# lunarring/latentblending

Measured on AMD Instinct MI355X. Metric: transition frames/sec, SDXL-Turbo 512x512 4-step 15-branch, higher is better.
Workload: dtype f16; 1 GPU; SDXL-Turbo 512x512, num_inference_steps=4, nmb_max_branches=15 (17 frames/transition), fp16, fixed_seeds=[420,421], anchors not recycled; frontier_width=16, hipgraphs=True, parallelism=single GPU

## Files before the change

### include/lb_hip.h

```cpp
#ifndef LB_HIP_H
#define LB_HIP_H

#include <stdint.h>

#ifdef __cplusplus
extern "C" {
#endif

typedef uint16_t lb_half;

int lb_version(void);
const char* lb_last_error_string(void);
int lb_device_info(int device, int* cu_count, long* lds_per_cu, char* arch, int arch_len);

int lb_slerp_pairs_f16(const void* const* p0, const void* const* p1, void* const* out,
                       const double* fracts, int npairs, long n, void* stream);
int lb_slerp_pairs_f32(const void* const* p0, const void* const* p1, void* const* out,
                       const double* fracts, int npairs, long n, void* stream);
int lb_slerp_pairs_f64(const void* const* p0, const void* const* p1, void* const* out,
                       const double* fracts, int npairs, long n, void* stream);
int lb_slerp_batched_f16(const void* p0, const void* p1, void* out, const double* fracts_dev,
                         long npairs, long n, void* stream);
int lb_slerp_strided_f16(const void* p0, long stride0, const void* p1, long stride1, void* out,
                         const double* fracts_dev, long npairs, long n, void* stream);
// ... 9 lines not shown
                      void* stream);
int lb_ddim_step_f16(const void* x, const void* eps, void* out, const float* params_dev, long per_sample, int batch,
                     int cfg, void* stream);

enum {
    LB_GEMM_OUT_F32 = 1,
    LB_GEMM_RES_F32 = 2,
    LB_GEMM_GEGLU = 4,
    LB_GEMM_TRANS_OUT = 8,
    LB_GEMM_SILU = 16,
    LB_GEMM_RELU = 32,
    LB_GEMM_QUICK_GELU = 128,
    LB_GEMM_GELU = 256,
    LB_GEMM_CH_STATS = 512,
    LB_GEMM_HALO_RAGGED = 1024,
    LB_GEMM_C64 = 2048,
    LB_GEMM_LN_A = 64
};

typedef struct LbGemmParams {
    const lb_half* A;
    const lb_half* W;
    void* C;
    const float* bias;
    const void* residual;
    const lb_half* rowvec;
    float* partial;
    int M, N, K;
    int lda, ldw, ldc, ldr, ld_rowvec, rows_per_batch;
    float alpha;
// ... 11 lines not shown
    float* ch_stats;
    int ch_stats_rows;
} LbGemmParams;

int lb_gemm_f16(const LbGemmParams* params, void* stream);
long lb_gemm_workspace_bytes(int M, int N);
void lb_gemm_set_tuning(int tile, int splitk);
void lb_gemm_set_pp_auto(int on);
void lb_gemm_pp_set_group(int gm);
void lb_gemm_set_depth(int depth);
int lb_gemm_plan(const LbGemmParams* p, int* tile, int* splitk, long* blocks);
int lb_conv3x3_halo_f16(const LbGemmParams* params, void* stream);
int lb_conv3x3_narrow_f16(const LbGemmParams* params, void* stream);
void lb_conv_halo_set_persistent(int on);
void lb_conv_halo_plan(const LbGemmParams* params, int* kind, int* tile_w, long* items, long* grid);
int lb_gemm_ch_stat_rows(const LbGemmParams* params);
int lb_upconv2x_halo_f16(const LbGemmParams* params, void* stream);
void lb_gemm_set_halo(int mode);
void lb_gemm_set_wide_store(int on);
void lb_gemm_set_t192_waves8(int on);
void lb_gemm_set_kgroups(int on);
void lb_gemm_set_lean_epilogue(int on);
void lb_gemm_set_variant(int variant, int stages);

void lb_groupnorm_set_l3_chunk(long bytes);
int lb_groupnorm_from_stats(const void* x, void* y, const float* gamma, const float* beta, const float* ch_stats,
                            void* workspace, int B, int HW, int C, int ldx, int ldy, int groups, float eps, int silu,
                            int x_is_f32, int stat_rows_per_sample, void* stream);
long lb_groupnorm_workspace_bytes(int B, int groups);
int lb_groupnorm_nhwc(const void* x, void* y, const float* gamma, const float* beta, void* workspace,
// ... 81 lines not shown
```

### latentblending_amd/csrc/conv3_halo.hip

```cpp
#include <type_traits>
#include "lb_common.h"
#include "lb_gemm.h"

typedef __attribute__((address_space(1))) const void* gptr_t;
typedef __attribute__((address_space(3))) void* lptr_t;

#ifndef LB_HALO_LEAN_ADDR
#define LB_HALO_LEAN_ADDR 1
#endif

template <int N> __device__ __forceinline__ void halo_wait_barrier() {
    asm volatile("s_waitcnt vmcnt(%0)\n\ts_barrier" ::"n"(N) : "memory");
}

template <int KS, int J> struct HaloSched {
    static constexpr int tap = KS == 3 ? J : (J < 3 ? 0 : 1);
};
template <int KS, int NR, int TAP> constexpr int halo_full_rounds_in_tap() {
    int n = 0;
    for (int j = 0; j < NR - 1; ++j) n += ((KS == 3 ? j : (j < 3 ? 0 : 1)) == TAP) ? 1 : 0;
    return n;
}

template <int BN, int TW, int KS = 3, bool RAG = false>
__global__ void __launch_bounds__(512) conv3x3_halo_kernel(const LbGemmParams p) {
    static_assert(!RAG || KS == 3, "ragged tiles exist for the 3x3 form only");
    constexpr int TH = 256 / TW;
    constexpr int NTAP = KS * KS;
    constexpr int HWP = TW + KS - 1;
    constexpr int HR = (TH + KS - 1) * HWP;
    constexpr int HRG = (HR + 7) / 8;
    constexpr int HRP = HRG * 8;
    constexpr int NR = (HRG + 7) / 8;
    constexpr int EXTRA = HRG - 8 * (NR - 1);
    constexpr int WI = BN * 8 / 512;
    constexpr int TM = 4, TN = BN / 32;
    static_assert(NR == (KS == 3 ? 6 : 5), "halo rounds: 6 for the 3x3 form, 5 for the 2x2 form");
    static_assert(EXTRA >= 1 && EXTRA <= 8, "the last halo round is a partial one");
    static_assert(WI == 2, "the vmcnt schedule assumes two weight loads per thread and step");
    extern __shared__ __attribute__((aligned(16))) f16 lds[];
    f16* const halo0 = lds;
// ... 1 lines not shown

    const int tid = threadIdx.x, lane = tid & 63;
    const int wave = LB_HALO_LEAN_ADDR ? __builtin_amdgcn_readfirstlane(tid >> 6) : tid >> 6;
    const int wave_m = wave >> 1, wave_n = wave & 1;
    const int g = lane >> 4, l16 = lane & 15;

    const int n_blocks = (p.N + BN - 1) / BN;
    const int tiles_x = RAG ? (p.Win + TW - 1) / TW : p.Win / TW, tiles_y = RAG ? (p.Hin + TH - 1) / TH : p.Hin / TH;
    const int n_items = (p.M / (p.Hin * p.Win)) * tiles_x * tiles_y * (KS == 2 ? 4 : 1) * n_blocks;
    const int G = gridDim.x;
    int bid = blockIdx.x;
    {
        const int q = G / 8, r = G % 8, xcd = bid % 8, idx = bid / 8;
        bid = (xcd < r ? xcd * (q + 1) : r * (q + 1) + (xcd - r) * q) + idx;
    }
    const int block_n = bid % n_blocks;
    const int par_x = KS == 2 ? (bid / n_blocks) & 1 : 0;
    const int par_y = KS == 2 ? ((bid / n_blocks) >> 1) & 1 : 0;
    const int n0 = block_n * BN;
    const int org_y = KS == 3 ? 1 : 1 - par_y, org_x = KS == 3 ? 1 : 1 - par_x;
    const lb_half* Wp = p.W + (KS == 2 ? (long)(par_y * 2 + par_x) * p.N * p.ldw : 0);
    const int nchunks = p.Cin / 64;
    const lb_half* zero = reinterpret_cast<const lb_half*>(p.zero_page);

    struct TileAt { int b, y0, x0; };
    auto tile_of = [&](int item) {
        int tile = item / n_blocks;
        if (KS == 2) tile >>= 2;
        TileAt t;
        t.x0 = (tile % tiles_x) * TW;
        tile /= tiles_x;
        t.y0 = (tile % tiles_y) * TH;
        t.b = tile / tiles_y;
        return t;
    };

    const int r8 = lane >> 3;
    const int cl = (lane & 7) ^ r8;
    long h_off[NR];
    auto set_halo_offsets = [&](const TileAt& t, bool exists) {
#pragma unroll
        for (int j = 0; j < NR; ++j) {
            const int gidx = j * 8 + wave;
            const int row = gidx * 8 + r8;
            const int hy = row / HWP, hx = row - hy * HWP;
            const int y = t.y0 + hy - org_y, x = t.x0 + hx - org_x;
            const bool ok = exists && (j < NR - 1 || wave < EXTRA) && row < HR && y >= 0 && y < p.Hin && x >= 0 && x < p.Win;
            h_off[j] = ok ? ((long)(t.b * p.Hin + y) * p.Win + x) * p.ldx + cl * 8 : -1;
        }
    };
    long w_off[WI];
    unsigned w_off32[WI];
#pragma unroll
    for (int i = 0; i < WI; ++i) {
        const int n = n0 + (tid >> 3) + i * 64;
        w_off[i] = n < p.N ? (long)n * p.ldw + cl * 8 : -1;
        w_off32[i] = (unsigned)(((long)(n < p.N ? n : p.N - 1) * p.ldw + cl * 8) * 2);
    }

#ifdef LB_STUDY_BUILD
    const int study = p.reserved_;
#else
    constexpr int study = 0;
#endif
    auto issue_halo = [&](int j, int src_chunk, int buf) {
        const lb_half* src = h_off[j] >= 0 && !(study & 2) ? p.A + h_off[j] + (long)src_chunk * 64 : zero;
        const int gidx = j * 8 + wave;
        f16* dst = halo0 + buf * (HRP * 64) + gidx * 8 * 64;
        __builtin_amdgcn_global_load_lds((gptr_t)src, (lptr_t)dst, 16, 0, 0);
    };
    auto issue_weight = [&](int i, int chunk, bool exists, int tap, int slot) {
        f16* dst = wring + slot * (BN * 64) + (wave * 8 + i * 64) * 64;
        if constexpr (LB_HALO_LEAN_ADDR) {
            if (!(study & 4)) {
                const char* base = reinterpret_cast<const char*>(Wp) + ((long)tap * p.Cin + (long)chunk * 64) * 2;
                __builtin_amdgcn_global_load_lds((gptr_t)(base + (size_t)w_off32[i]), (lptr_t)dst, 16, 0, 0);
                return;
            }
        }
        const bool live = w_off[i] >= 0 && exists && !(study & 4);
        const lb_half* src = live ? Wp + w_off[i] + (long)tap * p.Cin + (long)chunk * 64 : zero;
        __builtin_amdgcn_global_load_lds((gptr_t)src, (lptr_t)dst, 16, 0, 0);
    };

    int hbase[TM];
    int mloc[TM];
#pragma unroll
    for (int i = 0; i < TM; ++i) {
        const int m = wave_m * 64 + i * 16 + l16;
        const int py = m / TW, px = m - py * TW;
        hbase[i] = py * HWP + px;
        mloc[i] = py * p.Win + px;
    }
    f32x4 acc[TM][TN];
#pragma unroll
    for (int i = 0; i < TM; ++i)
// ... 20 lines not shown
        }
#pragma unroll
        for (int j = 0; j < TN; ++j) {
            const int r = j * 16 + l16;
            wf[j] = *reinterpret_cast<const f16x8*>(wb + (wave_n * (BN / 2) + r) * 64 + ((chunk ^ (r & 7)) << 3));
        }
    };
    auto mma_rows = [&](const f16x8 (&af)[TM], const f16x8 (&wf)[TN], int i_lo, int i_hi) {
#pragma unroll
        for (int i = i_lo; i < i_hi; ++i)
#pragma unroll
            for (int j = 0; j < TN; ++j)
                acc[i][j] = __builtin_amdgcn_mfma_f32_16x16x32_f16(wf[j], af[i], acc[i][j], 0, 0, 0);
    };

    int item = bid;
    TileAt cur = tile_of(item);
    set_halo_offsets(cur, true);
#pragma unroll
    for (int j = 0; j < NR; ++j)
        if (j < NR - 1 || wave < EXTRA) issue_halo(j, 0, 0);
#pragma unroll
    for (int t = 0; t < 3; ++t)
#pragma unroll
        for (int i = 0; i < WI; ++i) issue_weight(i, 0, true, t, t);

    auto step = [&](auto tap_c, int c, int cc, bool more) {
        constexpr int TAP = decltype(tap_c)::value;
        constexpr int P1 = (TAP + NTAP - 1) % NTAP, P2 = (TAP + NTAP - 2) % NTAP;
        constexpr int CNT = (2 + halo_full_rounds_in_tap<KS, NR, P1>()) + (2 + halo_full_rounds_in_tap<KS, NR, P2>());
        halo_wait_barrier<CNT>();
        const int slot = KS == 3 ? ((cc + TAP) & 3) : TAP;
        const f16* hb = halo0 + (cc & 1) * (HRP * 64);
        const f16* wb = wring + slot * (BN * 64);
        constexpr int KY = TAP / KS, KX = TAP % KS;
        int shift = KY * HWP + KX;
        asm volatile("" : "+v"(shift));
        const bool last = c + 1 == nchunks;
        const int hc = last ? 0 : c + 1, hbuf = (cc + 1) & 1;
        constexpr int TAP3 = (TAP + 3) % NTAP;
        const bool wrap = (TAP + 3 >= NTAP) && last;
        const int c3 = wrap ? 0 : c + (TAP + 3) / NTAP;
        const bool w_exists = !wrap || more;
        const int slot3 = (slot + 3) & 3;
        f16x8 a0[TM], w0[TN], a1[TM], w1[TN];
        read_frags(hb, wb, shift, 0, a0, w0);
        if constexpr (HaloSched<KS, 0>::tap == TAP) issue_halo(0, hc, hbuf);
        if constexpr (NR > 2 && HaloSched<KS, 1>::tap == TAP) issue_halo(1, hc, hbuf);
        if constexpr (NR > 3 && HaloSched<KS, 2>::tap == TAP) issue_halo(2, hc, hbuf);
        if constexpr (NR > 4 && HaloSched<KS, 3>::tap == TAP) { if (NR - 1 > 3 || wave < EXTRA) issue_halo(3, hc, hbuf); }
        if constexpr (NR > 4 && HaloSched<KS, 4>::tap == TAP) { if (NR - 1 > 4 || wave < EXTRA) issue_halo(4, hc, hbuf); }
        if constexpr (NR > 5 && HaloSched<KS, 5>::tap == TAP) { if (wave < EXTRA) issue_halo(5, hc, hbuf); }
        __builtin_amdgcn_sched_barrier(0);
        mma_rows(a0, w0, 0, TM / 2);
        read_frags(hb, wb, shift, 1, a1, w1);
        __builtin_amdgcn_sched_barrier(0);
        issue_weight(0, c3, w_exists, TAP3, slot3);
        __builtin_amdgcn_sched_barrier(0);
        mma_rows(a0, w0, TM / 2, TM);
        __builtin_amdgcn_sched_barrier(0);
        issue_weight(1, c3, w_exists, TAP3, slot3);
        __builtin_amdgcn_sched_barrier(0);
        mma_rows(a1, w1, 0, TM);
    };

    LbGemmParams q = p;
    if constexpr (KS == 2) {
        q.scatter = 1;
        q.sc_py = par_y;
        q.sc_px = par_x;
    }

    int cc = 0;
    for (;;) {
        const int next_item = item + G;
        const bool more = next_item < n_items;
        const TileAt nxt = tile_of(more ? next_item : item);
        for (int c = 0; c < nchunks; ++c, ++cc) {
            if (c + 1 == nchunks) set_halo_offsets(nxt, more);
            step(std::integral_constant<int, 0>{}, c, cc, more);
            step(std::integral_constant<int, 1>{}, c, cc, more);
            step(std::integral_constant<int, 2>{}, c, cc, more);
            step(std::integral_constant<int, 3>{}, c, cc, more);
            if constexpr (KS == 3) {
                step(std::integral_constant<int, 4>{}, c, cc, more);
                step(std::integral_constant<int, 5>{}, c, cc, more);
                step(std::integral_constant<int, 6>{}, c, cc, more);
                step(std::integral_constant<int, 7>{}, c, cc, more);
                step(std::integral_constant<int, 8>{}, c, cc, more);
            }
        }
        const int mbase = (cur.b * p.Hin + cur.y0) * p.Win + cur.x0;
        int col0 = n0 + wave_n * (BN / 2) + 4 * g;
        asm volatile("" : "+v"(col0));
        bool overhang = false;
        if constexpr (RAG) overhang = cur.y0 + TH > p.Hin || cur.x0 + TW > p.Win;
        if (RAG && overhang && !(study & 1)) {
            int tid_o = tid;
            asm volatile("" : "+v"(tid_o));
            auto row_of = [&](int i) {
                const int ml = (tid_o >> 7) * 64 + i * 16 + (tid_o & 15), ly = ml / TW, lx = ml - ly * TW;
                return cur.y0 + ly < p.Hin && cur.x0 + lx < p.Win ? mbase + mloc[i] : p.M;
            };
            if (p.flags & LB_GEMM_CH_STATS) {
                const long stat_rows = (long)(n_items / n_blocks) * 4;
                float2* chst = reinterpret_cast<float2*>(p.ch_stats) + ((long)(item / n_blocks) * 4 + wave_m);
                lb_gemm_tile_epilogue_rows_ln<TM, TN, false, false, true, true>(q, acc, row_of, col0, 0, (const LbLnRows<TM>*)nullptr, chst, stat_rows);
            } else {
                lb_gemm_tile_epilogue_rows<TM, TN, false>(q, acc, row_of, col0, 0);
            }
        } else if (!(study & 1)) {
            int tid_o = tid;
            asm volatile("" : "+v"(tid_o));
            auto out_rel = [&](int i) {
                if constexpr (KS == 3) return mloc[i];
                const int ml = (tid_o >> 7) * 64 + i * 16 + (tid_o & 15), ly = ml / TW, lx = ml - ly * TW;
                return 4 * ly * p.Win + 2 * lx;
            };
            const long out_lo = KS == 3 ? (long)mbase
                                        : ((long)(cur.b * 2 * p.Hin + 2 * cur.y0 + par_y)) * (2 * p.Win) + 2 * cur.x0 + par_x;
            const int row_hi = mbase + (TH - 1) * p.Win + TW;
            const int colw = col0 - 4 * ((tid_o & 63) >> 4);
            if (p.flags & LB_GEMM_CH_STATS) {
                const long stat_rows = (long)(n_items / n_blocks) * 4;
                float2* chst = reinterpret_cast<float2*>(p.ch_stats) + ((long)(item / n_blocks) * 4 + wave_m);
                if (!lb_gemm_tile_epilogue_lean<TM, TN, true, true>(q, acc, [&](int i) { return mbase + mloc[i]; }, mbase, row_hi, out_rel,
                                                                    out_lo, cur.b, colw, chst, stat_rows))
                    lb_gemm_tile_epilogue_rows_ln<TM, TN, false, false, true>(q, acc, [&](int i) { return mbase + mloc[i]; }, col0, 0,
                                                                              (const LbLnRows<TM>*)nullptr, chst, stat_rows);
            } else {
                if (!lb_gemm_tile_epilogue_lean<TM, TN, false, true>(q, acc, [&](int i) { return mbase + mloc[i]; }, mbase, row_hi, out_rel,
                                                                     out_lo, cur.b, colw))
                    lb_gemm_tile_epilogue_rows<TM, TN, false>(q, acc, [&](int i) { return mbase + mloc[i]; }, col0, 0);
            }
        }
        else if (acc[0][0][0] == 12345.678f) *(float*)p.C = acc[1][1][1] + acc[2][2][2] + acc[3][3][3];
        if (!more) break;
#pragma unroll
        for (int i = 0; i < TM; ++i)
#pragma unroll
            for (int j = 0; j < TN; ++j) acc[i][j] = (f32x4){0.f, 0.f, 0.f, 0.f};
        item = next_item;
        cur = nxt;
    }
    asm volatile("s_waitcnt vmcnt(0)" ::: "memory");
}

static int g_halo_persistent = 1;
extern "C" void lb_conv_halo_set_persistent(int on) { g_halo_persistent = on; }
#ifdef LB_STUDY_BUILD
static int g_halo_study = 0;
extern "C" void lb_conv_halo_set_study(int bits) { g_halo_study = bits; }
#endif
static int halo_num_cus() {
    static int n = 0;
    if (!n) {
        int dev = 0;
        hipDeviceProp_t prop;
// ... 14 lines not shown
        grid = (long)(halo_num_cus() / period) * period;
}

int lb_upconv_halo_eligible(const LbGemmParams& p);
int lb_conv3x3_halo_eligible(const LbGemmParams& p);
long lb_conv_halo_stat_rows_total(const LbGemmParams& p) {
    int tw = 0, ks = 0;
    if ((tw = lb_upconv_halo_eligible(p)) != 0) ks = 2;
    else if ((tw = lb_conv3x3_halo_eligible(p)) != 0) ks = 3;
    if (!ks) return 0;
    long items, grid;
    halo_grid(p, tw, ks, items, grid);
    return items / ((p.N + 127) / 128) * 4;
}

template <int BN, int TW, int KS = 3, bool RAG = false>
static int launch_halo(const LbGemmParams& p, hipStream_t stream) {
    constexpr int TH = 256 / TW;
    constexpr int HRP = (((TH + KS - 1) * (TW + KS - 1) + 7) / 8) * 8;
    constexpr int SMEM = (2 * HRP * 64 + 4 * BN * 64) * (int)sizeof(f16);
    static unsigned long long seen = 0;
    LB_ONCE_PER_DEVICE(seen)
        (void)hipFuncSetAttribute(reinterpret_cast<const void*>(conv3x3_halo_kernel<BN, TW, KS, RAG>),
                                  hipFuncAttributeMaxDynamicSharedMemorySize, SMEM);
    static_assert(BN == 128, "halo_grid assumes 128-channel blocks");
    long nblk, grid;
    halo_grid(p, TW, KS, nblk, grid);
    LbGemmParams pk = p;
#ifdef LB_STUDY_BUILD
    pk.reserved_ = g_halo_study;
#endif
    hipLaunchKernelGGL((conv3x3_halo_kernel<BN, TW, KS, RAG>), dim3((unsigned)grid), dim3(512), SMEM, stream, pk);
    return lb_check_launch(KS == 2 ? "lb_upconv2x_halo_f16" : "lb_conv3x3_halo_f16");
}

int lb_upconv_halo_eligible(const LbGemmParams& p) {
    if (!p.conv || p.scatter != 2 || p.KH != 2 || p.KW != 2 || p.stride != 1 || p.ups) return 0;
    if (p.Hout != p.Hin || p.Wout != p.Win || p.Cin % 64 != 0 || p.K != 4 * p.Cin) return 0;
    if (p.zero_page == nullptr || (p.flags & (LB_GEMM_GEGLU | LB_GEMM_TRANS_OUT)) || p.N % 4 != 0 || p.residual != nullptr) return 0;
    if (p.M % (p.Hin * p.Win) != 0) return 0;
    if ((long)p.N * p.ldw * 2 >= (1l << 32)) return 0;
    if (p.Win % 32 == 0 && p.Hin % 8 == 0) return 32;
    if (p.Win % 16 == 0 && p.Hin % 16 == 0) return 16;
    return 0;
}

static int halo_tiles_check(const LbGemmParams& p, int tw, int ks) {
// ... 30 lines not shown

int lb_conv3x3_halo_eligible(const LbGemmParams& p) {
    if (!p.conv || p.KH != 3 || p.KW != 3 || p.stride != 1 || p.pad != 1 || p.ups || p.scatter) return 0;
    if (p.Hout != p.Hin || p.Wout != p.Win || p.Cin % 64 != 0 || p.K != 9 * p.Cin) return 0;
    if (p.zero_page == nullptr || (p.flags & LB_GEMM_GEGLU) || p.N % 4 != 0) return 0;
    if (p.M % (p.Hin * p.Win) != 0) return 0;
    if ((long)p.N * p.ldw * 2 >= (1l << 32)) return 0;
    if (p.Win % 32 == 0 && p.Hin % 8 == 0) return 32;
    if (p.Win % 16 == 0 && p.Hin % 16 == 0) return 16;
    if (!(p.flags & LB_GEMM_HALO_RAGGED)) return 0;
    const long t32 = (long)((p.Win + 31) / 32) * ((p.Hin + 7) / 8), t16 = (long)((p.Win + 15) / 16) * ((p.Hin + 15) / 16);
    return t16 < t32 ? 16 : 32;
}
static bool halo3_ragged(const LbGemmParams& p, int tw) { return p.Win % tw != 0 || p.Hin % (256 / tw) != 0; }

long lb_conv3x3_halo_blocks(const LbGemmParams& p) {
    long tiles = (long)p.M / 256;
    if (const int tw = (p.flags & LB_GEMM_HALO_RAGGED) ? lb_conv3x3_halo_eligible(p) : 0)
        tiles = (long)(p.M / (p.Hin * p.Win)) * ((p.Hin + 256 / tw - 1) / (256 / tw)) * ((p.Win + tw - 1) / tw);
    return tiles * ((p.N + 127) / 128);
}

int lb_conv3x3_halo_check(const LbGemmParams& p) {
    LB_REQUIRE(!(p.flags & LB_GEMM_CH_STATS) || (p.ch_stats != nullptr && !(p.flags & LB_GEMM_TRANS_OUT)),
               "halo conv: LB_GEMM_CH_STATS needs ch_stats and a row-major output");
    LB_REQUIRE(!(p.flags & LB_GEMM_CH_STATS) || p.ch_stats_rows == lb_conv_halo_stat_rows_total(p),
               "halo conv: ch_stats_rows must be B * lb_gemm_ch_stat_rows() (the row blocks this launch writes per channel)");
    return halo_tiles_check(p, lb_conv3x3_halo_eligible(p), 3);
}

int lb_conv3x3_halo_launch(LbGemmParams p, hipStream_t stream) {
    if (p.alpha == 0.f) p.alpha = 1.f;
    p.splitk = 1;
    const int tw = lb_conv3x3_halo_eligible(p);
    if (halo3_ragged(p, tw)) return tw == 32 ? launch_halo<128, 32, 3, true>(p, stream) : launch_halo<128, 16, 3, true>(p, stream);
    return tw == 32 ? launch_halo<128, 32>(p, stream) : launch_halo<128, 16>(p, stream);
}

extern "C" int lb_conv3x3_halo_f16(const LbGemmParams* pp, void* stream) {
    LbGemmParams p = *pp;
    p.flags &= ~LB_GEMM_C64;
    p.reserved2_ = (g_lb_wide_store & 1) | (g_lb_lean_epilogue ? 2 : 0);
    LB_REQUIRE(p.M > 0 && p.N > 0 && p.K > 0, "lb_conv3x3_halo_f16: empty problem");
    LB_REQUIRE(lb_conv3x3_halo_eligible(p) != 0,
               "lb_conv3x3_halo_f16: needs a 3x3 / stride 1 / pad 1 conv, Cin % 64 == 0, W % 16 == 0 (or LB_GEMM_HALO_RAGGED), zero page");
    LB_REQUIRE(p.ldw % 8 == 0 && p.ldx % 8 == 0 && (p.ldc % 4 == 0 || (p.flags & LB_GEMM_TRANS_OUT)),
               "lb_conv3x3_halo_f16: ldw / ldx multiples of 8, ldc multiple of 4");
    if (const int rc = lb_conv3x3_halo_check(p)) return rc;
    LB_DISPATCH("lb_conv3x3_halo_f16", lb_conv3x3_halo_launch(p, s));
}
// ... 15 lines not shown
```

### latentblending_amd/csrc/gemm.hip

```cpp
#include "lb_common.h"
#include "lb_gemm.h"

#define BK 64

template <int N> struct Int { static constexpr int value = N; };

template <int BM, int BN, bool CONV, bool GEGLU, int D>
__global__ void __launch_bounds__(256) gemm_f16_kernel(const LbGemmParams p) {
    constexpr int AI = BM * 8 / 256;
    constexpr int WI = BN * 8 / 256;
    constexpr int TM = BM / 32;
    constexpr int TN = BN / 32;
    __shared__ __attribute__((aligned(16))) f16 lds[2 * (BM + BN) * BK];
    f16* const As = lds;
    f16* const Ws = lds + 2 * BM * BK;

    const int tid = threadIdx.x;
    const int lane = tid & 63, wave = tid >> 6;
    const int wave_m = wave >> 1, wave_n = wave & 1;
    const int g = lane >> 4, l16 = lane & 15;

    const int n_blocks = GEGLU ? (p.N / 2 + BN / 2 - 1) / (BN / 2) : (p.N + BN - 1) / BN;
    int bid = blockIdx.x;
    {
// ... 471 lines not shown
        LB_DISPATCH("conv3x3_c64", lb_conv3_c64_launch(p, s));
    }
    if (p.scatter == 2) {
        LB_REQUIRE(lb_upconv_halo_eligible(p) != 0, "lb_gemm_f16: scatter = 2 needs Cin % 64 == 0, W % 16 == 0, stacked [4][N][K] weights");
        if (const int rc = lb_upconv_halo_check(p)) return rc;
        LB_DISPATCH("lb_upconv2x_halo_f16", lb_upconv_halo_launch(p, s));
    }
    if (g_halo != 0 && !g_force_tile && lb_conv3x3_narrow_eligible(p)) {
        if (const int rc = lb_conv3x3_narrow_check(p)) return rc;
        LB_DISPATCH("lb_conv3x3_narrow_f16", lb_conv3x3_narrow_launch(p, s));
    }
    if (use_halo(p)) {
        if (const int rc = lb_conv3x3_halo_check(p)) return rc;
        LB_DISPATCH("lb_conv3x3_halo_f16", lb_conv3x3_halo_launch(p, s));
    }
    LB_REQUIRE(!(p.flags & LB_GEMM_CH_STATS), "lb_gemm_f16: LB_GEMM_CH_STATS is implemented by the halo-tile conv kernels only "
                                              "(check lb_gemm_plan == 6 / lb_conv_halo_plan before asking for it)");
    int tile = 0, splitk = 1;
    long nblk = 0;
    gemm_plan(p, tile, splitk, nblk);
    p.splitk = splitk;
    const int depth = g_depth, variant = g_variant;
    int stages = g_stages;
    if (variant == 1) {
        lb_gemm_glds_init();
        if (stages == 0)
            stages = (tile == 3 || tile == 4 || tile == 7 || tile == 10 || tile == 11) ? 3 : 2;
    }
    const dim3 grid((unsigned)nblk, 1, (unsigned)splitk);
    LB_DISPATCH("lb_gemm_f16", gemm_launch_impl(p, tile, depth, variant, stages, grid, s));
// ... 2 lines not shown
```

### latentblending_amd/hip/lib.py

```python
from __future__ import annotations

import ctypes as C
import os

import torch

_HERE = os.path.dirname(os.path.abspath(__file__))
LIB_PATH = os.environ.get("LB_HIP_LIBRARY") or os.path.join(_HERE, "liblbhip.so")

c_void_pp = C.POINTER(C.c_void_p)


class LbGemmParams(C.Structure):
    _fields_ = [
        ("A", C.c_void_p), ("W", C.c_void_p), ("C", C.c_void_p), ("bias", C.c_void_p),
        ("residual", C.c_void_p), ("rowvec", C.c_void_p), ("partial", C.c_void_p),
        ("M", C.c_int), ("N", C.c_int), ("K", C.c_int),
        ("lda", C.c_int), ("ldw", C.c_int), ("ldc", C.c_int), ("ldr", C.c_int),
        ("ld_rowvec", C.c_int), ("rows_per_batch", C.c_int),
        ("alpha", C.c_float), ("flags", C.c_int),
        ("conv", C.c_int), ("Hin", C.c_int), ("Win", C.c_int), ("Cin", C.c_int),
        ("Hout", C.c_int), ("Wout", C.c_int), ("KH", C.c_int), ("KW", C.c_int),
        ("stride", C.c_int), ("pad", C.c_int), ("ups", C.c_int), ("ldx", C.c_int),
        ("splitk", C.c_int), ("zero_page", C.c_void_p),
# ... 2 lines not shown
    ]


class LbAttnParams(C.Structure):
    _fields_ = [
        ("Q", C.c_void_p), ("K", C.c_void_p), ("V", C.c_void_p), ("O", C.c_void_p),
        ("B", C.c_int), ("H", C.c_int), ("Sq", C.c_int), ("Skv", C.c_int), ("Skv_valid", C.c_int),
        ("ldq", C.c_int), ("ldk", C.c_int), ("ldv", C.c_int), ("ldo", C.c_int),
        ("scale", C.c_float), ("causal", C.c_int), ("zero_page", C.c_void_p), ("reserved_", C.c_int),
    ]


GEMM_OUT_F32, GEMM_RES_F32, GEMM_GEGLU, GEMM_TRANS_OUT, GEMM_SILU, GEMM_RELU, GEMM_LN_A = 1, 2, 4, 8, 16, 32, 64
GEMM_QUICK_GELU, GEMM_GELU, GEMM_CH_STATS = 128, 256, 512
GEMM_HALO_RAGGED = 1024
GEMM_C64 = 2048

_vp, _i, _l, _f, _d = C.c_void_p, C.c_int, C.c_long, C.c_float, C.c_double

SIGNATURES = {
    "lb_version": (_i, []),
    "lb_last_error_string": (C.c_char_p, []),
    "lb_device_info": (_i, [_i, C.POINTER(_i), C.POINTER(_l), C.c_char_p, _i]),
    "lb_slerp_pairs_f16": (_i, [c_void_pp, c_void_pp, c_void_pp, C.POINTER(_d), _i, _l, _vp]),
    "lb_slerp_pairs_f32": (_i, [c_void_pp, c_void_pp, c_void_pp, C.POINTER(_d), _i, _l, _vp]),
    "lb_slerp_pairs_f64": (_i, [c_void_pp, c_void_pp, c_void_pp, C.POINTER(_d), _i, _l, _vp]),
    "lb_slerp_batched_f16": (_i, [_vp, _vp, _vp, _vp, _l, _l, _vp]),
    "lb_slerp_strided_f16": (_i, [_vp, _l, _vp, _l, _vp, _vp, _l, _l, _vp]),
    "lb_lerp_f16": (_i, [_vp, _vp, _vp, _l, _d, _vp]),
    "lb_lerp_f32": (_i, [_vp, _vp, _vp, _l, _d, _vp]),
# ... 59 lines not shown
    "lb_program_num_ops": (_i, [_vp]),
    "lb_program_op_name": (C.c_char_p, [_vp, _i]),
    "lb_program_run": (_i, [_vp, _vp]),
    "lb_program_run_range": (_i, [_vp, _i, _i, _vp]),
    "lb_program_instantiate": (_i, [_vp]),
    "lb_program_launch": (_i, [_vp, _vp]),
    "lb_program_time_ops": (_i, [_vp, _vp, C.POINTER(C.c_float)]),
}

STUDY_SIGNATURES = {
    "lb_slerp_set_study": (None, [_i]),
    "lb_gemm_set_policy": (None, [_i]),
    "lb_conv_halo_set_study": (None, [_i]),
}

_NO_CHECK = {"lb_version", "lb_last_error_string", "lb_gemm_workspace_bytes", "lb_jpeg_coefficient_count", "lb_jpeg_workspace_bytes",
             "lb_groupnorm_workspace_bytes", "lb_groupnorm_set_l3_chunk", "lb_conv_halo_set_persistent", "lb_conv_halo_plan", "lb_gemm_ch_stat_rows", "lb_conv_halo_set_study", "lb_gemm_set_tuning", "lb_gemm_set_depth", "lb_gemm_set_variant", "lb_gemm_set_wide_store", "lb_gemm_set_lean_epilogue", "lb_gemm_set_t192_waves8", "lb_gemm_set_kgroups", "lb_gemm_pp_set_group", "lb_gemm_set_pp_auto", "lb_gemm_set_policy", "lb_gemm_set_halo", "lb_attn_set_tuning", "lb_layernorm_set_form", "lb_groupnorm_set_fused", "lb_groupnorm_plan", "lb_slerp_set_study", "lb_program_create",
             "lb_program_destroy", "lb_program_recording", "lb_program_num_ops", "lb_program_op_name"}


def _load():
    if not os.path.isfile(LIB_PATH):
        raise ImportError(
            f"latentblending_amd: {LIB_PATH} is missing. Build it with "
            "`python -c 'import __graft_entry__ as g; g.build()'` (hipcc, gfx950). "
            "There is no CPU fallback for the kernel path.")
    return C.CDLL(LIB_PATH, mode=C.RTLD_GLOBAL)


_lib = _load()


# ... 6 lines not shown
        rc = fn(*args)
        if rc != 0:
            msg = _lib.lb_last_error_string()
            raise RuntimeError(f"{name} failed ({rc}): {msg.decode() if msg else '?'}")
        return rc
    checked.__name__ = name
    return checked


api = _Api()
for _name, (_res, _args) in SIGNATURES.items():
    _fn = getattr(_lib, _name)
    _fn.restype = _res
    _fn.argtypes = _args
    setattr(api, _name, _fn if _name in _NO_CHECK else _wrap(_name, _fn))
for _name, (_res, _args) in STUDY_SIGNATURES.items():
    _fn = getattr(_lib, _name, None)
    if _fn is not None:
        _fn.restype = _res
        _fn.argtypes = _args
        setattr(api, _name, _fn)

if os.environ.get("LB_GEMM_WIDE_STORE"):
    api.lb_gemm_set_wide_store(int(os.environ["LB_GEMM_WIDE_STORE"]))
if os.environ.get("LB_GEMM_LEAN_EPILOGUE"):
    api.lb_gemm_set_lean_epilogue(int(os.environ["LB_GEMM_LEAN_EPILOGUE"]))
if os.environ.get("LB_GEMM_PP_AUTO"):
    api.lb_gemm_set_pp_auto(int(os.environ["LB_GEMM_PP_AUTO"]))
```

### latentblending_amd/native/runtime.py

```python
from __future__ import annotations

import contextlib
import ctypes as C
from typing import Dict, List, Optional, Tuple

import torch

from ..hip import lib
from ..hip.lib import api, LbGemmParams, LbAttnParams
from .geometry import use_ragged_halo

F16, F32 = torch.float16, torch.float32


class Arena:
    def __init__(self, device):
        self.device = device
        self.free: Dict[int, List[torch.Tensor]] = {}
        self.all: List[torch.Tensor] = []
        self.bytes_allocated = 0

    @staticmethod
    def _cls(nbytes: int) -> int:
        return max(512, (nbytes + 511) // 512 * 512)
# ... 89 lines not shown


class Emitter:

    def __init__(self, arena: Arena):
        self.arena = arena
        self.device = arena.device
        self.ws_gemm: Optional[torch.Tensor] = None
        self.ws_gn: Optional[torch.Tensor] = None
        self.gemm_log: List[dict] = []
        self.attn_log: List[dict] = []
        self.norm_log: List[dict] = []
        self._retired: List[torch.Tensor] = []
        self.zero_page = torch.zeros(64, dtype=torch.uint8, device=self.device)
        self.ragged_halo = False

    def _ragged_flag(self, p: LbGemmParams) -> int:
        if not self.ragged_halo or not p.conv or p.KH != 3 or p.KW != 3 or p.stride != 1 or p.scatter or p.ups or p.N <= 16:
            return 0
        kind, tw = C.c_int(), C.c_int()
        flags = p.flags
        p.flags = flags & ~lib.GEMM_HALO_RAGGED
        api.lb_conv_halo_plan(C.byref(p), C.byref(kind), None, None, None)
        plain = kind.value
        p.flags = flags | lib.GEMM_HALO_RAGGED
        api.lb_conv_halo_plan(C.byref(p), C.byref(kind), C.byref(tw), None, None)
        p.flags = flags
        return lib.GEMM_HALO_RAGGED if use_ragged_halo(True, plain, kind.value, p.Hin, p.Win, tw.value) else 0

    def _gemm_ws(self, M: int, N: int) -> Optional[torch.Tensor]:
        if ((M + 63) // 64) * ((N + 63) // 64) > 640:
            return None
        need = api.lb_gemm_workspace_bytes(M, N) // 4
        if self.ws_gemm is None or self.ws_gemm.numel() < need:
            if self.ws_gemm is not None:
                self._retired.append(self.ws_gemm)
            self.ws_gemm = torch.empty(max(need, 1 << 22), dtype=F32, device=self.device)
        return self.ws_gemm

    def _gn_ws(self, B: int, groups: int) -> torch.Tensor:
        need = api.lb_groupnorm_workspace_bytes(B, groups) // 8
        if self.ws_gn is None or self.ws_gn.numel() < need:
            if self.ws_gn is not None:
                self._retired.append(self.ws_gn)
            self.ws_gn = torch.empty(need, dtype=torch.float64, device=self.device)
        return self.ws_gn

    def gemm(self, A: torch.Tensor, W: torch.Tensor, out: torch.Tensor, *, M: int, bias=None,
             residual=None, rowvec=None, rows_per_batch: int = 0, flags: int = 0, alpha: float = 1.0,
             lda: Optional[int] = None, ldc: Optional[int] = None, ldr: Optional[int] = None,
             ld_rowvec: Optional[int] = None, conv: Optional[dict] = None, splitk: bool = True,
             ln: Optional[Tuple[torch.Tensor, float]] = None, ch_stats: Optional[torch.Tensor] = None):
        p = LbGemmParams()
# ... 17 lines not shown
        if rowvec is not None:
            p.ld_rowvec, p.rows_per_batch = ld_rowvec if ld_rowvec is not None else N, rows_per_batch
        p.alpha, p.flags = alpha, flags
        p.zero_page = self.zero_page.data_ptr()
        if ln is not None:
            p.flags |= lib.GEMM_LN_A
            p.ln_colsum, p.ln_eps = ln[0].data_ptr(), float(ln[1])
        if ch_stats is not None:
            assert conv is not None and ch_stats.dtype == F32
            p.flags |= lib.GEMM_CH_STATS
            p.ch_stats, p.ch_stats_rows = ch_stats.data_ptr(), ch_stats.shape[1]
        if splitk and not (flags & lib.GEMM_GEGLU) and ln is None:
            p.partial = _p(self._gemm_ws(M, N))
        if self.ragged_halo:
            p.flags |= self._ragged_flag(p)
        api.lb_gemm_f16(C.byref(p), _stream())
        mult = 4.0 if p.scatter == 2 else 1.0
        self.gemm_log.append({"M": M, "N": N, "K": K, "flops": mult * 2.0 * M * N * K, "conv": conv is not None,
                              "bytes": mult * 2.0 * (N * K + M * n_out) + (2.0 * M * K if conv is None else 0.0)})
        return out

    def plan(self, M: int, N: int, K: int, flags: int = 0) -> Tuple[int, int]:
        p = LbGemmParams()
        p.M, p.N, p.K, p.flags = M, N, K, flags
        p.zero_page = self.zero_page.data_ptr()
        if not (flags & lib.GEMM_GEGLU):
            p.partial = _p(self._gemm_ws(M, N))
        t, sk, nb = C.c_int(), C.c_int(), C.c_long()
        api.lb_gemm_plan(C.byref(p), C.byref(t), C.byref(sk), C.byref(nb))
        return t.value, sk.value
# ... 62 lines not shown
```

Before: 124.1 frames/s.

## Add stream-K style split of the input-channel loop for halo 3x3 convs

Adds a K-split variant of the persistent halo 3x3 conv kernel. Work is divided into (tile, 64-channel chunk) units spread evenly over a CU-sized grid. Blocks that hold a partial tile write fp32 accumulators to slabs and bump an atomic counter, and the last block to arrive reduces the slabs and runs the epilogue. The goal is to remove tail-wave load imbalance when the number of tiles does not divide evenly across CUs. The cost is extra slab traffic, atomics and a fixup reduction, and a host-side plan decides per conv whether splitting is worth it.

New measurement: 126.1 frames/s, median of 6. +1.6%, better.

```diff
diff --git a/include/lb_hip.h b/include/lb_hip.h
--- a/include/lb_hip.h
+++ b/include/lb_hip.h
@@ -47,6 +47,7 @@
     LB_GEMM_GELU = 256,
     LB_GEMM_CH_STATS = 512,
     LB_GEMM_HALO_RAGGED = 1024,
+    LB_GEMM_HALO_KSPLIT = 4096,
     LB_GEMM_C64 = 2048,
     LB_GEMM_LN_A = 64
 };
@@ -88,6 +89,7 @@
 int lb_conv3x3_narrow_f16(const LbGemmParams* params, void* stream);
 void lb_conv_halo_set_persistent(int on);
 void lb_conv_halo_plan(const LbGemmParams* params, int* kind, int* tile_w, long* items, long* grid);
+#include "lb_hip_ksplit.h"
 int lb_gemm_ch_stat_rows(const LbGemmParams* params);
 int lb_upconv2x_halo_f16(const LbGemmParams* params, void* stream);
 void lb_gemm_set_halo(int mode);
diff --git a/include/lb_hip_ksplit.h b/include/lb_hip_ksplit.h
--- /dev/null
+++ b/include/lb_hip_ksplit.h
@@ -0,0 +1,12 @@
+#ifndef LB_HIP_KSPLIT_H
+#define LB_HIP_KSPLIT_H
+#ifdef __cplusplus
+extern "C" {
+#endif
+void lb_conv_halo_ksplit_plan(const LbGemmParams* params, long* units, long* grid, int* split);
+long lb_conv_halo_ksplit_workspace_bytes(const LbGemmParams* params);
+void lb_conv_halo_set_ksplit(int mode, int grid);
+#ifdef __cplusplus
+}
+#endif
+#endif
diff --git a/latentblending_amd/csrc/conv3_halo.hip b/latentblending_amd/csrc/conv3_halo.hip
--- a/latentblending_amd/csrc/conv3_halo.hip
+++ b/latentblending_amd/csrc/conv3_halo.hip
@@ -22,9 +22,10 @@
     return n;
 }
 
-template <int BN, int TW, int KS = 3, bool RAG = false>
+template <int BN, int TW, int KS = 3, bool RAG = false, bool KSP = false>
 __global__ void __launch_bounds__(512) conv3x3_halo_kernel(const LbGemmParams p) {
     static_assert(!RAG || KS == 3, "ragged tiles exist for the 3x3 form only");
+    static_assert(!KSP || (KS == 3 && !RAG), "the K-split form exists for the whole-tile 3x3 form only");
     constexpr int TH = 256 / TW;
     constexpr int NTAP = KS * KS;
     constexpr int HWP = TW + KS - 1;
@@ -56,10 +57,16 @@
         const int q = G / 8, r = G % 8, xcd = bid % 8, idx = bid / 8;
         bid = (xcd < r ? xcd * (q + 1) : r * (q + 1) + (xcd - r) * q) + idx;
     }
-    const int block_n = bid % n_blocks;
+    const int n_tiles = KSP ? n_items / n_blocks : 0;
+    const long n_units = KSP ? (long)n_items * (p.Cin / 64) : 0;
+    const long u_lo = KSP ? (long)bid * n_units / G : 0, u_hi = KSP ? (long)(bid + 1) * n_units / G : 0;
+    if constexpr (KSP)
+        if (u_lo >= u_hi) return;
+    const int first_item = KSP ? (int)(u_lo / (p.Cin / 64)) : bid;
+    const int block_n = KSP ? first_item / n_tiles : bid % n_blocks;
     const int par_x = KS == 2 ? (bid / n_blocks) & 1 : 0;
     const int par_y = KS == 2 ? ((bid / n_blocks) >> 1) & 1 : 0;
-    const int n0 = block_n * BN;
+    int n0 = block_n * BN;
     const int org_y = KS == 3 ? 1 : 1 - par_y, org_x = KS == 3 ? 1 : 1 - par_x;
     const lb_half* Wp = p.W + (KS == 2 ? (long)(par_y * 2 + par_x) * p.N * p.ldw : 0);
     const int nchunks = p.Cin / 64;
@@ -67,7 +74,7 @@
 
     struct TileAt { int b, y0, x0; };
     auto tile_of = [&](int item) {
-        int tile = item / n_blocks;
+        int tile = KSP ? item % n_tiles : item / n_blocks;
         if (KS == 2) tile >>= 2;
         TileAt t;
         t.x0 = (tile % tiles_x) * TW;
@@ -91,14 +98,18 @@
             h_off[j] = ok ? ((long)(t.b * p.Hin + y) * p.Win + x) * p.ldx + cl * 8 : -1;
         }
     };
-    long w_off[WI];
-    unsigned w_off32[WI];
-#pragma unroll
-    for (int i = 0; i < WI; ++i) {
-        const int n = n0 + (tid >> 3) + i * 64;
-        w_off[i] = n < p.N ? (long)n * p.ldw + cl * 8 : -1;
-        w_off32[i] = (unsigned)(((long)(n < p.N ? n : p.N - 1) * p.ldw + cl * 8) * 2);
-    }
+    long w_off[WI], w_offn[WI];
+    unsigned w_off32[WI], w_off32n[WI];
+    auto set_w_offsets = [&](int col_base, long (&o64)[WI], unsigned (&o32)[WI]) {
+#pragma unroll
+        for (int i = 0; i < WI; ++i) {
+            const int n = col_base + (tid >> 3) + i * 64;
+            o64[i] = n < p.N ? (long)n * p.ldw + cl * 8 : -1;
+            o32[i] = (unsigned)(((long)(n < p.N ? n : p.N - 1) * p.ldw + cl * 8) * 2);
+        }
+    };
+    set_w_offsets(n0, w_off, w_off32);
+    if constexpr (KSP) set_w_offsets(n0, w_offn, w_off32n);
 
 #ifdef LB_STUDY_BUILD
     const int study = p.reserved_;
@@ -111,17 +122,19 @@
         f16* dst = halo0 + buf * (HRP * 64) + gidx * 8 * 64;
         __builtin_amdgcn_global_load_lds((gptr_t)src, (lptr_t)dst, 16, 0, 0);
     };
-    auto issue_weight = [&](int i, int chunk, bool exists, int tap, int slot) {
+    auto issue_weight = [&](int i, int chunk, bool exists, int tap, int slot, bool nxt_slab = false) {
         f16* dst = wring + slot * (BN * 64) + (wave * 8 + i * 64) * 64;
         if constexpr (LB_HALO_LEAN_ADDR) {
             if (!(study & 4)) {
                 const char* base = reinterpret_cast<const char*>(Wp) + ((long)tap * p.Cin + (long)chunk * 64) * 2;
-                __builtin_amdgcn_global_load_lds((gptr_t)(base + (size_t)w_off32[i]), (lptr_t)dst, 16, 0, 0);
+                const unsigned o32 = KSP && nxt_slab ? w_off32n[i] : w_off32[i];
+                __builtin_amdgcn_global_load_lds((gptr_t)(base + (size_t)o32), (lptr_t)dst, 16, 0, 0);
                 return;
             }
         }
-        const bool live = w_off[i] >= 0 && exists && !(study & 4);
-        const lb_half* src = live ? Wp + w_off[i] + (long)tap * p.Cin + (long)chunk * 64 : zero;
+        const long o64 = KSP && nxt_slab ? w_offn[i] : w_off[i];
+        const bool live = o64 >= 0 && exists && !(study & 4);
+        const lb_half* src = live ? Wp + o64 + (long)tap * p.Cin + (long)chunk * 64 : zero;
         __builtin_amdgcn_global_load_lds((gptr_t)src, (lptr_t)dst, 16, 0, 0);
     };
 
@@ -172,16 +185,21 @@
                 acc[i][j] = __builtin_amdgcn_mfma_f32_16x16x32_f16(wf[j], af[i], acc[i][j], 0, 0, 0);
     };
 
-    int item = bid;
+    int item = first_item;
+    int c_lo = 0, c_end = nchunks;
+    if constexpr (KSP) {
+        c_lo = (int)(u_lo - (long)item * nchunks);
+        c_end = (int)(u_hi - (long)item * nchunks < nchunks ? u_hi - (long)item * nchunks : nchunks);
+    }
     TileAt cur = tile_of(item);
     set_halo_offsets(cur, true);
 #pragma unroll
     for (int j = 0; j < NR; ++j)
-        if (j < NR - 1 || wave < EXTRA) issue_halo(j, 0, 0);
+        if (j < NR - 1 || wave < EXTRA) issue_halo(j, c_lo, 0);
 #pragma unroll
     for (int t = 0; t < 3; ++t)
 #pragma unroll
-        for (int i = 0; i < WI; ++i) issue_weight(i, 0, true, t, t);
+        for (int i = 0; i < WI; ++i) issue_weight(i, c_lo, true, t, t);
 
     auto step = [&](auto tap_c, int c, int cc, bool more) {
         constexpr int TAP = decltype(tap_c)::value;
@@ -194,7 +212,7 @@
         constexpr int KY = TAP / KS, KX = TAP % KS;
         int shift = KY * HWP + KX;
         asm volatile("" : "+v"(shift));
-        const bool last = c + 1 == nchunks;
+        const bool last = c + 1 == c_end;
         const int hc = last ? 0 : c + 1, hbuf = (cc + 1) & 1;
         constexpr int TAP3 = (TAP + 3) % NTAP;
         const bool wrap = (TAP + 3 >= NTAP) && last;
@@ -213,11 +231,11 @@
         mma_rows(a0, w0, 0, TM / 2);
         read_frags(hb, wb, shift, 1, a1, w1);
         __builtin_amdgcn_sched_barrier(0);
-        issue_weight(0, c3, w_exists, TAP3, slot3);
+        issue_weight(0, c3, w_exists, TAP3, slot3, wrap);
         __builtin_amdgcn_sched_barrier(0);
         mma_rows(a0, w0, TM / 2, TM);
         __builtin_amdgcn_sched_barrier(0);
-        issue_weight(1, c3, w_exists, TAP3, slot3);
+        issue_weight(1, c3, w_exists, TAP3, slot3, wrap);
         __builtin_amdgcn_sched_barrier(0);
         mma_rows(a1, w1, 0, TM);
     };
@@ -231,11 +249,15 @@
 
     int cc = 0;
     for (;;) {
-        const int next_item = item + G;
-        const bool more = next_item < n_items;
+        const int next_item = KSP ? item + 1 : item + G;
+        const bool more = KSP ? (long)next_item * nchunks < u_hi : next_item < n_items;
         const TileAt nxt = tile_of(more ? next_item : item);
-        for (int c = 0; c < nchunks; ++c, ++cc) {
-            if (c + 1 == nchunks) set_halo_offsets(nxt, more);
+        const int n0_next = KSP && more ? (next_item / n_tiles) * BN : n0;
+        for (int c = c_lo; c < c_end; ++c, ++cc) {
+            if (c + 1 == c_end) {
+                set_halo_offsets(nxt, more);
+                if constexpr (KSP) set_w_offsets(n0_next, w_offn, w_off32n);
+            }
             step(std::integral_constant<int, 0>{}, c, cc, more);
             step(std::integral_constant<int, 1>{}, c, cc, more);
             step(std::integral_constant<int, 2>{}, c, cc, more);
@@ -246,6 +268,68 @@
                 step(std::integral_constant<int, 6>{}, c, cc, more);
                 step(std::integral_constant<int, 7>{}, c, cc, more);
                 step(std::integral_constant<int, 8>{}, c, cc, more);
+            }
+        }
+        if constexpr (KSP) {
+            if (c_lo != 0 || c_end != nchunks) {
+                const long t0 = (long)item * nchunks;
+                const int b_first = (int)(((t0 + 1) * G - 1) / n_units), b_last = (int)(((t0 + nchunks) * G - 1) / n_units);
+                constexpr long SLAB = 256l * BN;
+                int* const counters = reinterpret_cast<int*>(p.partial);
+                float* const slabs = p.partial + (((long)n_items * 4 + 255) / 256) * 64;
+                int tid_s = tid;
+                asm volatile("" : "+v"(tid_s));
+                typedef unsigned u32x4 __attribute__((ext_vector_type(4)));
+                const __amdgpu_buffer_rsrc_t srs = __builtin_amdgcn_make_buffer_rsrc(slabs, 0, (int)(unsigned)(2l * G * SLAB * 4), 0x00020000);
+                const int voff = tid_s * 16;
+                const int mine = (2 * bid + (item == first_item ? 0 : 1)) * (int)(SLAB * 4);
+#pragma unroll
+                for (int i = 0; i < TM; ++i)
+#pragma unroll
+                    for (int j = 0; j < TN; ++j)
+                        __builtin_amdgcn_raw_buffer_store_b128(__builtin_bit_cast(u32x4, acc[i][j]), srs, voff, mine + (i * TN + j) * 8192, 16);
+                volatile int* const flag = reinterpret_cast<volatile int*>(lds + 2 * HRP * 64 + 4 * BN * 64);
+                asm volatile("s_waitcnt vmcnt(0)" ::: "memory");
+                __syncthreads();
+                if (tid == 0) {
+                    const int ticket = __hip_atomic_fetch_add(counters + item, 1, __ATOMIC_RELAXED, __HIP_MEMORY_SCOPE_AGENT);
+                    const bool last_one = ticket == b_last - b_first;
+                    if (last_one) __hip_atomic_store(counters + item, 0, __ATOMIC_RELAXED, __HIP_MEMORY_SCOPE_AGENT);
+                    *flag = last_one ? 1 : 0;
+                }
+                __syncthreads();
+                const bool reduce = __builtin_amdgcn_readfirstlane(*flag) != 0;
+                if (!reduce) {
+                    if (!more) break;
+#pragma unroll
+                    for (int i = 0; i < TM; ++i)
+#pragma unroll
+                        for (int j = 0; j < TN; ++j) acc[i][j] = (f32x4){0.f, 0.f, 0.f, 0.f};
+                    item = next_item;
+                    cur = nxt;
+                    n0 = n0_next;
+                    set_w_offsets(n0, w_off, w_off32);
+                    c_lo = 0;
+                    c_end = (int)(u_hi - (long)item * nchunks < nchunks ? u_hi - (long)item * nchunks : nchunks);
+                    continue;
+                }
+#pragma unroll
+                for (int i = 0; i < TM; ++i)
+#pragma unroll
+                    for (int j = 0; j < TN; ++j) acc[i][j] = (f32x4){0.f, 0.f, 0.f, 0.f};
+                for (int b = b_first; b <= b_last; ++b) {
+                    const bool first_tile_of_b = (long)b * n_units / G / nchunks == item;
+                    const int src = (2 * b + (first_tile_of_b ? 0 : 1)) * (int)(SLAB * 4);
+#pragma unroll
+                    for (int i = 0; i < TM; ++i) {
+                        f32x4 part[TN];
+#pragma unroll
+                        for (int j = 0; j < TN; ++j)
+                            part[j] = __builtin_bit_cast(f32x4, __builtin_amdgcn_raw_buffer_load_b128(srs, voff, src + (i * TN + j) * 8192, 16));
+#pragma unroll
+                        for (int j = 0; j < TN; ++j) acc[i][j] += part[j];
+                    }
+                }
             }
         }
         const int mbase = (cur.b * p.Hin + cur.y0) * p.Win + cur.x0;
@@ -262,7 +346,7 @@
             };
             if (p.flags & LB_GEMM_CH_STATS) {
                 const long stat_rows = (long)(n_items / n_blocks) * 4;
-                float2* chst = reinterpret_cast<float2*>(p.ch_stats) + ((long)(item / n_blocks) * 4 + wave_m);
+                float2* chst = reinterpret_cast<float2*>(p.ch_stats) + ((long)(KSP ? item % n_tiles : item / n_blocks) * 4 + wave_m);
                 lb_gemm_tile_epilogue_rows_ln<TM, TN, false, false, true, true>(q, acc, row_of, col0, 0, (const LbLnRows<TM>*)nullptr, chst, stat_rows);
             } else {
                 lb_gemm_tile_epilogue_rows<TM, TN, false>(q, acc, row_of, col0, 0);
@@ -281,7 +365,7 @@
             const int colw = col0 - 4 * ((tid_o & 63) >> 4);
             if (p.flags & LB_GEMM_CH_STATS) {
                 const long stat_rows = (long)(n_items / n_blocks) * 4;
-                float2* chst = reinterpret_cast<float2*>(p.ch_stats) + ((long)(item / n_blocks) * 4 + wave_m);
+                float2* chst = reinterpret_cast<float2*>(p.ch_stats) + ((long)(KSP ? item % n_tiles : item / n_blocks) * 4 + wave_m);
                 if (!lb_gemm_tile_epilogue_lean<TM, TN, true, true>(q, acc, [&](int i) { return mbase + mloc[i]; }, mbase, row_hi, out_rel,
                                                                     out_lo, cur.b, colw, chst, stat_rows))
                     lb_gemm_tile_epilogue_rows_ln<TM, TN, false, false, true>(q, acc, [&](int i) { return mbase + mloc[i]; }, col0, 0,
@@ -300,6 +384,12 @@
             for (int j = 0; j < TN; ++j) acc[i][j] = (f32x4){0.f, 0.f, 0.f, 0.f};
         item = next_item;
         cur = nxt;
+        if constexpr (KSP) {
+            n0 = n0_next;
+            set_w_offsets(n0, w_off, w_off32);
+            c_lo = 0;
+            c_end = (int)(u_hi - (long)item * nchunks < nchunks ? u_hi - (long)item * nchunks : nchunks);
+        }
     }
     asm volatile("s_waitcnt vmcnt(0)" ::: "memory");
 }
@@ -344,23 +434,24 @@
     return items / ((p.N + 127) / 128) * 4;
 }
 
-template <int BN, int TW, int KS = 3, bool RAG = false>
-static int launch_halo(const LbGemmParams& p, hipStream_t stream) {
+template <int BN, int TW, int KS = 3, bool RAG = false, bool KSP = false>
+static int launch_halo(const LbGemmParams& p, hipStream_t stream, long ksp_grid = 0) {
     constexpr int TH = 256 / TW;
     constexpr int HRP = (((TH + KS - 1) * (TW + KS - 1) + 7) / 8) * 8;
-    constexpr int SMEM = (2 * HRP * 64 + 4 * BN * 64) * (int)sizeof(f16);
+    constexpr int SMEM = (2 * HRP * 64 + 4 * BN * 64) * (int)sizeof(f16) + (KSP ? 16 : 0);
     static unsigned long long seen = 0;
     LB_ONCE_PER_DEVICE(seen)
-        (void)hipFuncSetAttribute(reinterpret_cast<const void*>(conv3x3_halo_kernel<BN, TW, KS, RAG>),
+        (void)hipFuncSetAttribute(reinterpret_cast<const void*>(conv3x3_halo_kernel<BN, TW, KS, RAG, KSP>),
                                   hipFuncAttributeMaxDynamicSharedMemorySize, SMEM);
     static_assert(BN == 128, "halo_grid assumes 128-channel blocks");
     long nblk, grid;
     halo_grid(p, TW, KS, nblk, grid);
+    if (KSP) grid = ksp_grid;
     LbGemmParams pk = p;
 #ifdef LB_STUDY_BUILD
     pk.reserved_ = g_halo_study;
 #endif
-    hipLaunchKernelGGL((conv3x3_halo_kernel<BN, TW, KS, RAG>), dim3((unsigned)grid), dim3(512), SMEM, stream, pk);
+    hipLaunchKernelGGL((conv3x3_halo_kernel<BN, TW, KS, RAG, KSP>), dim3((unsigned)grid), dim3(512), SMEM, stream, pk);
     return lb_check_launch(KS == 2 ? "lb_upconv2x_halo_f16" : "lb_conv3x3_halo_f16");
 }
 
@@ -421,6 +512,55 @@
 }
 static bool halo3_ragged(const LbGemmParams& p, int tw) { return p.Win % tw != 0 || p.Hin % (256 / tw) != 0; }
 
+static int g_halo_ksplit_mode = 1, g_halo_ksplit_grid = 0;
+extern "C" void lb_conv_halo_set_ksplit(int mode, int grid) {
+    g_halo_ksplit_mode = mode < 0 ? 1 : mode;
+    g_halo_ksplit_grid = grid > 0 ? grid : 0;
+}
+static constexpr long HALO_KSPLIT_FIXUP_STEPS = 20;
+static constexpr long HALO_KSPLIT_MARGIN_PCT = 5;
+static void halo_ksplit_plan(const LbGemmParams& p, long& units, long& grid, int& split) {
+    units = grid = 0;
+    split = 0;
+    if (!(p.flags & LB_GEMM_HALO_KSPLIT) || (p.flags & LB_GEMM_C64) || g_halo_ksplit_mode == 0) return;
+    const int tw = lb_conv3x3_halo_eligible(p);
+    if (!tw || halo3_ragged(p, tw) || p.Cin < 128) return;
+    long items, ugrid;
+    halo_grid(p, tw, 3, items, ugrid);
+    const long nchunks = p.Cin / 64;
+    if (items * nchunks >= (1l << 31)) return;
+    units = items * nchunks;
+    grid = g_halo_ksplit_grid > 0 ? g_halo_ksplit_grid : halo_num_cus();
+    if (grid > units) grid = units;
+    if (2 * grid * 256l * 128 * 4 >= (1l << 31)) {
+        units = grid = 0;
+        return;
+    }
+    if (g_halo_ksplit_mode >= 2) {
+        split = 1;
+        return;
+    }
+    const long unsplit_steps = (items + ugrid - 1) / ugrid * 9 * nchunks;
+    const long split_steps = (units + grid - 1) / grid * 9 + HALO_KSPLIT_FIXUP_STEPS;
+    split = split_steps * (100 + HALO_KSPLIT_MARGIN_PCT) <= unsplit_steps * 100 ? 1 : 0;
+}
+static long halo_ksplit_counter_bytes(long items) { return (items * 4 + 255) / 256 * 256; }
+extern "C" void lb_conv_halo_ksplit_plan(const LbGemmParams* pp, long* units, long* grid, int* split) {
+    long u = 0, g = 0;
+    int s = 0;
+    if (pp != nullptr && pp->M > 0 && pp->Hin > 0 && pp->Win > 0) halo_ksplit_plan(*pp, u, g, s);
+    if (units) *units = u;
+    if (grid) *grid = g;
+    if (split) *split = s;
+}
+extern "C" long lb_conv_halo_ksplit_workspace_bytes(const LbGemmParams* pp) {
+    long u = 0, g = 0;
+    int s = 0;
+    if (pp != nullptr && pp->M > 0 && pp->Hin > 0 && pp->Win > 0) halo_ksplit_plan(*pp, u, g, s);
+    if (!s) return 0;
+    return halo_ksplit_counter_bytes(u / (pp->Cin / 64)) + 2 * g * 256l * 128 * (long)sizeof(float);
+}
+
 long lb_conv3x3_halo_blocks(const LbGemmParams& p) {
     long tiles = (long)p.M / 256;
     if (const int tw = (p.flags & LB_GEMM_HALO_RAGGED) ? lb_conv3x3_halo_eligible(p) : 0)
@@ -433,6 +573,13 @@
                "halo conv: LB_GEMM_CH_STATS needs ch_stats and a row-major output");
     LB_REQUIRE(!(p.flags & LB_GEMM_CH_STATS) || p.ch_stats_rows == lb_conv_halo_stat_rows_total(p),
                "halo conv: ch_stats_rows must be B * lb_gemm_ch_stat_rows() (the row blocks this launch writes per channel)");
+    {
+        long units, grid;
+        int split;
+        halo_ksplit_plan(p, units, grid, split);
+        LB_REQUIRE(!split || p.partial != nullptr,
+                   "halo conv: LB_GEMM_HALO_KSPLIT needs partial = a zeroed workspace of lb_conv_halo_ksplit_workspace_bytes()");
+    }
     return halo_tiles_check(p, lb_conv3x3_halo_eligible(p), 3);
 }
 
@@ -441,6 +588,11 @@
     p.splitk = 1;
     const int tw = lb_conv3x3_halo_eligible(p);
     if (halo3_ragged(p, tw)) return tw == 32 ? launch_halo<128, 32, 3, true>(p, stream) : launch_halo<128, 16, 3, true>(p, stream);
+    long units, grid;
+    int split;
+    halo_ksplit_plan(p, units, grid, split);
+    if (split && p.partial != nullptr)
+        return tw == 32 ? launch_halo<128, 32, 3, false, true>(p, stream, grid) : launch_halo<128, 16, 3, false, true>(p, stream, grid);
     return tw == 32 ? launch_halo<128, 32>(p, stream) : launch_halo<128, 16>(p, stream);
 }
 
diff --git a/latentblending_amd/csrc/gemm.hip b/latentblending_amd/csrc/gemm.hip
--- a/latentblending_amd/csrc/gemm.hip
+++ b/latentblending_amd/csrc/gemm.hip
@@ -509,6 +509,10 @@
         if (const int rc = lb_conv3x3_halo_check(p)) return rc;
         LB_DISPATCH("lb_conv3x3_halo_f16", lb_conv3x3_halo_launch(p, s));
     }
+    if (p.flags & LB_GEMM_HALO_KSPLIT) {
+        p.flags &= ~LB_GEMM_HALO_KSPLIT;
+        p.partial = nullptr;
+    }
     LB_REQUIRE(!(p.flags & LB_GEMM_CH_STATS), "lb_gemm_f16: LB_GEMM_CH_STATS is implemented by the halo-tile conv kernels only "
                                               "(check lb_gemm_plan == 6 / lb_conv_halo_plan before asking for it)");
     int tile = 0, splitk = 1;
diff --git a/latentblending_amd/hip/lib.py b/latentblending_amd/hip/lib.py
--- a/latentblending_amd/hip/lib.py
+++ b/latentblending_amd/hip/lib.py
@@ -40,6 +40,7 @@
 GEMM_OUT_F32, GEMM_RES_F32, GEMM_GEGLU, GEMM_TRANS_OUT, GEMM_SILU, GEMM_RELU, GEMM_LN_A = 1, 2, 4, 8, 16, 32, 64
 GEMM_QUICK_GELU, GEMM_GELU, GEMM_CH_STATS = 128, 256, 512
 GEMM_HALO_RAGGED = 1024
+GEMM_HALO_KSPLIT = 4096
 GEMM_C64 = 2048
 
 _vp, _i, _l, _f, _d = C.c_void_p, C.c_int, C.c_long, C.c_float, C.c_double
@@ -129,8 +130,14 @@
     "lb_conv_halo_set_study": (None, [_i]),
 }
 
+HOST_SIGNATURES = {
+    "lb_conv_halo_ksplit_plan": (None, [C.POINTER(LbGemmParams), C.POINTER(C.c_long), C.POINTER(C.c_long), C.POINTER(C.c_int)]),
+    "lb_conv_halo_ksplit_workspace_bytes": (_l, [C.POINTER(LbGemmParams)]),
+    "lb_conv_halo_set_ksplit": (None, [_i, _i]),
+}
+
 _NO_CHECK = {"lb_version", "lb_last_error_string", "lb_gemm_workspace_bytes", "lb_jpeg_coefficient_count", "lb_jpeg_workspace_bytes",
-             "lb_groupnorm_workspace_bytes", "lb_groupnorm_set_l3_chunk", "lb_conv_halo_set_persistent", "lb_conv_halo_plan", "lb_gemm_ch_stat_rows", "lb_conv_halo_set_study", "lb_gemm_set_tuning", "lb_gemm_set_depth", "lb_gemm_set_variant", "lb_gemm_set_wide_store", "lb_gemm_set_lean_epilogue", "lb_gemm_set_t192_waves8", "lb_gemm_set_kgroups", "lb_gemm_pp_set_group", "lb_gemm_set_pp_auto", "lb_gemm_set_policy", "lb_gemm_set_halo", "lb_attn_set_tuning", "lb_layernorm_set_form", "lb_groupnorm_set_fused", "lb_groupnorm_plan", "lb_slerp_set_study", "lb_program_create",
+             "lb_groupnorm_workspace_bytes", "lb_groupnorm_set_l3_chunk", "lb_conv_halo_set_persistent", "lb_conv_halo_plan","lb_gemm_ch_stat_rows", "lb_conv_halo_set_study", "lb_gemm_set_tuning", "lb_gemm_set_depth", "lb_gemm_set_variant", "lb_gemm_set_wide_store", "lb_gemm_set_lean_epilogue", "lb_gemm_set_t192_waves8", "lb_gemm_set_kgroups", "lb_gemm_pp_set_group", "lb_gemm_set_pp_auto", "lb_gemm_set_policy", "lb_gemm_set_halo", "lb_attn_set_tuning", "lb_layernorm_set_form", "lb_groupnorm_set_fused", "lb_groupnorm_plan", "lb_slerp_set_study", "lb_program_create",
              "lb_program_destroy", "lb_program_recording", "lb_program_num_ops", "lb_program_op_name"}
 
 
@@ -167,6 +174,11 @@
     _fn.restype = _res
     _fn.argtypes = _args
     setattr(api, _name, _fn if _name in _NO_CHECK else _wrap(_name, _fn))
+for _name, (_res, _args) in HOST_SIGNATURES.items():
+    _fn = getattr(_lib, _name)
+    _fn.restype = _res
+    _fn.argtypes = _args
+    setattr(api, _name, _fn)
 for _name, (_res, _args) in STUDY_SIGNATURES.items():
     _fn = getattr(_lib, _name, None)
     if _fn is not None:
diff --git a/latentblending_amd/native/runtime.py b/latentblending_amd/native/runtime.py
--- a/latentblending_amd/native/runtime.py
+++ b/latentblending_amd/native/runtime.py
@@ -127,6 +127,8 @@
         self._retired: List[torch.Tensor] = []
         self.zero_page = torch.zeros(64, dtype=torch.uint8, device=self.device)
         self.ragged_halo = False
+        self.halo_ksplit = True
+        self.ws_ksplit: Optional[torch.Tensor] = None
 
     def _ragged_flag(self, p: LbGemmParams) -> int:
         if not self.ragged_halo or not p.conv or p.KH != 3 or p.KW != 3 or p.stride != 1 or p.scatter or p.ups or p.N <= 16:
@@ -150,6 +152,37 @@
                 self._retired.append(self.ws_gemm)
             self.ws_gemm = torch.empty(max(need, 1 << 22), dtype=F32, device=self.device)
         return self.ws_gemm
+
+    _KSPLIT_COUNTER_BYTES = 1 << 20
+
+    def _halo_ksplit(self, p: LbGemmParams) -> bool:
+        if not self.halo_ksplit or not p.conv or p.KH != 3 or p.KW != 3 or p.stride != 1 or p.scatter or p.ups:
+            return False
+        tile, sk, nb = C.c_int(), C.c_int(), C.c_long()
+        api.lb_gemm_plan(C.byref(p), C.byref(tile), C.byref(sk), C.byref(nb))
+        if tile.value != 6:
+            return False
+        flags = p.flags
+        p.flags = flags | lib.GEMM_HALO_KSPLIT
+        units, grid, split = C.c_long(), C.c_long(), C.c_int()
+        api.lb_conv_halo_ksplit_plan(C.byref(p), C.byref(units), C.byref(grid), C.byref(split))
+        need = int(api.lb_conv_halo_ksplit_workspace_bytes(C.byref(p)))
+        if not split.value or need <= 0:
+            p.flags = flags
+            return False
+        counters = ((units.value // (p.Cin // 64)) * 4 + 255) // 256 * 256
+        slabs = need - counters
+        assert slabs > 0 and slabs % (256 * 128 * 4) == 0, (need, counters)
+        if counters > self._KSPLIT_COUNTER_BYTES:
+            p.flags = flags
+            return False
+        total = self._KSPLIT_COUNTER_BYTES + slabs
+        if self.ws_ksplit is None or self.ws_ksplit.numel() < total:
+            if self.ws_ksplit is not None:
+                self._retired.append(self.ws_ksplit)
+            self.ws_ksplit = torch.zeros(total, dtype=torch.uint8, device=self.device)
+        p.partial = self.ws_ksplit.data_ptr() + self._KSPLIT_COUNTER_BYTES - counters
+        return True
 
     def _gn_ws(self, B: int, groups: int) -> torch.Tensor:
         need = api.lb_groupnorm_workspace_bytes(B, groups) // 8
@@ -197,6 +230,8 @@
             p.partial = _p(self._gemm_ws(M, N))
         if self.ragged_halo:
             p.flags |= self._ragged_flag(p)
+        if conv is not None:
+            self._halo_ksplit(p)
         api.lb_gemm_f16(C.byref(p), _stream())
         mult = 4.0 if p.scatter == 2 else 1.0
         self.gemm_log.append({"M": M, "N": N, "K": K, "flops": mult * 2.0 * M * N * K, "conv": conv is not None,
```
